# seobbro/TTA-depth-completion

Measured on AMD Instinct MI355X. Metric: TTA frames/sec (fwd+loss+bwd+Adam) at 352x1216, higher is better.
Workload: dtype mixed: real frames' forward (the scored depth) f32 storage + bf16x3 MFMA arithmetic; no_grad proxy pass and all data gradients bf16 storage + single bf16 MFMA; fp32 accumulate everywhere; loss / Adam / adapted parameters fp32 (include/ptta.h PTTA_DTYPE_MIXED)

## Files before the change

include/ptta.h:

```cpp
#ifndef PTTA_H
#define PTTA_H
#include <stdint.h>
#ifdef __cplusplus
extern "C" {
#endif

typedef struct ptta_ctx* ptta_handle;
typedef void* ptta_stream;

enum { PTTA_BACKBONE_MSG_CHN = 0, PTTA_BACKBONE_NLSPN = 1, PTTA_BACKBONE_COSTDCNET = 2 };
enum { PTTA_DTYPE_F32 = 0, PTTA_DTYPE_MIXED = 1,
       PTTA_MIXED_KEEP_PROXY = 0x100, PTTA_MIXED_KEEP_BACKWARD = 0x200, PTTA_MIXED_KEEP_HEADS = 0x400,
       PTTA_MIXED_BWD_ROUNDED_W = 0x800 };
enum { PTTA_META_1LAYER = 0, PTTA_META_2LAYERS = 1 };
enum { PTTA_NLSPN_LEGACY_OFFSET = 0x100,
       PTTA_NLSPN_SYNCBN_ADAPT = 0x200,
       PTTA_SYNCBN_ADAPT = 0x200 };

typedef struct {
    float lr, beta1, beta2, eps, weight_decay;
    float w_sparse_depth, w_smoothness, w_cos;
    float max_input_depth;
    float max_predict_depth;
} ptta_hparams;
// ... 76 lines not shown
int ptta_head_set_form(ptta_handle h, int form);

int ptta_crop_flip(const float* src, float* dst, int n, int channels, int height, int width, int crop_height, int crop_width,
                   const int32_t* start_y, const int32_t* start_x, const uint8_t* hflip, const uint8_t* vflip, ptta_stream s);

int ptta_rotate(const float* src, float* dst, int n, int channels, int height, int width, const uint8_t* do_rotate, const float* angle_deg,
                int bilinear, ptta_stream s);
int ptta_resize_crop(const float* src, float* dst, int n, int channels, int height, int width, const uint8_t* do_resize,
                     const int32_t* resize_height, const int32_t* resize_width, const int32_t* start_y, const int32_t* start_x,
                     int bilinear, int scale_depth, ptta_stream s);
int ptta_photometric(const float* src, float* dst, int n, int height, int width, const uint8_t* do_brightness, const float* f_brightness,
                     const uint8_t* do_contrast, const float* f_contrast, const uint8_t* do_saturation, const float* f_saturation,
                     double* scratch, ptta_stream s);

int ptta_photometric_full(const float* src, float* dst, int n, int height, int width, const uint8_t* do_brightness, const float* f_brightness,
                          const uint8_t* do_contrast, const float* f_contrast, const uint8_t* do_gamma, const float* f_gamma,
                          const uint8_t* do_hue, const float* f_hue, const uint8_t* do_saturation, const float* f_saturation,
                          double* scratch, ptta_stream s);
int ptta_add_noise(const float* src, const float* noise, float* dst, int n, int channels, int height, int width, const uint8_t* do_noise,
                   float spread, int uniform, ptta_stream s);
int ptta_remove_patches(const float* src, float* dst, int n, int channels, int height, int width, const uint8_t* do_remove,
                        const uint8_t* selected, const int32_t* patch_height, const int32_t* patch_width, ptta_stream s);
int ptta_crop_pad(const float* src, float* dst, int n, int channels, int height, int width, const uint8_t* do_crop_pad,
                  const int32_t* start_y, const int32_t* start_x, const int32_t* end_y, const int32_t* end_x,
                  const int32_t* pad_top, const int32_t* pad_left, int padding_mode, float fill, ptta_stream s);
int ptta_resize_pad(const float* src, float* dst, int n, int channels, int height, int width, const uint8_t* do_resize_pad,
                    const int32_t* resize_height, const int32_t* resize_width, const int32_t* pad_top, const int32_t* pad_left,
                    int bilinear, int padding_mode, float fill, ptta_stream s);

typedef int (*ptta_allreduce_fn)(void* user, double* exchange_buf, long long count, ptta_stream s);
int ptta_set_stat_sync(ptta_handle h, ptta_allreduce_fn fn, void* user, double* exchange_buf, int64_t capacity, int world_size);

int ptta_rccl_unique_id(void* id128_host);
int ptta_rccl_comm_create(const void* id128_host, int rank, int world_size, void** comm_out_host);
int ptta_rccl_comm_destroy(void* comm);
int ptta_rccl_allreduce_mean_f32(void* comm, float* buf, int64_t count, ptta_stream s);
const char* ptta_rccl_last_error(void);
int ptta_set_stat_sync_rccl(ptta_handle h, void* comm, double* exchange_buf, int64_t capacity, int world_size);
int ptta_set_grad_sync_rccl(ptta_handle h, void* comm);

int ptta_set_graph(ptta_handle h, int enable);

int ptta_set_option(ptta_handle h, const char* key, int value);
int ptta_get_option(ptta_handle h, const char* key, int* value_host);

int ptta_profile(ptta_handle h, int enable);
int ptta_profile_read(ptta_handle h, int klass, double* ms_total_host, double* alg_bytes_host, double* macs_host,
                      int64_t* launches_host, ptta_stream s);

int ptta_debug_tensor(ptta_handle h, const char* name, float* dst, int64_t capacity, int64_t* numel_host, ptta_stream s);
int ptta_op_conv32(const float* in_nhwc, const float* weight, const float* bias, float* out_nhwc,
                   int b, int hin, int win, int mode, int relu_in, int in_major, int flip, int dtype, int naive,
                   ptta_stream s);
int ptta_op_gwgrad(const float* x_nhwc, const float* gy_nhwc, float* gw, float* gb, int b, int h, int w, int ci, int co, int impl,
                   int reps, float* us_per_call_host, ptta_stream s);
#define PTTA_GCONV_S1 0
#define PTTA_GCONV_S2 1
#define PTTA_GCONV_T2 2
#define PTTA_GCONV_VERT 1
#define PTTA_GCONV_X1_W2 2
#define PTTA_GCONV_DGRAD 4
int ptta_op_gconv(const float* x0, int c0, int ld0, const float* x1, int c1, int ld1, const float* weight, const float* bias, float* y,
                  int co, int ldy, int b, int hin, int win, int hout, int wout, int k, int geom, int act, int accumulate, int impl,
                  int flags, int six_b, int x1_from_b, int stat_npass, double* stat_host, int* form_host, ptta_stream s);
#define PTTA_GBN_TRAIN 0
#define PTTA_GBN_EVAL 1
#define PTTA_GBN_BACKWARD 2
typedef struct ptta_gbn_view { float* p; int c; int ld; } ptta_gbn_view;
typedef struct ptta_gbn_args {
    int mode, b, h, w, npass, act, act_first, res_relu, acc_gx, acc_gres, world, nblocks_in, repeats;
    float eps, momentum;
    ptta_gbn_view x, res, y, g, gx, gres;
    const float* gamma; const float* beta; const float* part_in;
    float* st; float* rm; float* rv; long long* nbt; float* st_eval; float* dgamma; float* dbeta;
} ptta_gbn_args;
int ptta_op_gbn(const ptta_gbn_args* a, ptta_stream s);
int ptta_op_conv32_chain(const float* in_nhwc, const float* weight, const float* bias, float* buf_a, float* buf_b, const float* aux,
                         int b, int h, int w, int relu_in, int epi_flags, int reps, int replays, float* us_per_launch_host, ptta_stream s);
#define PTTA_ABI_VERSION 2
int ptta_version(void);

#ifdef __cplusplus
}
#endif
#endif
```

tta-depth-completion_amd/csrc/conv_small.hip:

```cpp
#include "ptta_common.h"
#include "ptta_kernels.h"

template <typename T>
struct ConvInP {
    Plane pl[3]; int zero_from_b;
    const float* w;
    Epi<T> epi;
    int B, H, W;
};

template <typename T, int CIN>
__global__ __launch_bounds__(256) void conv_in_mfma_kernel(ConvInP<T> p) {
    constexpr int K = 9 * CIN;
    constexpr int NS = (K + 1) / 2;
    const int lane = threadIdx.x & 63;
    const int i = lane & 31, h = lane >> 5;
    const int wave = __builtin_amdgcn_readfirstlane((int)(threadIdx.x >> 6));
    float w[NS];
#pragma unroll
    for (int s = 0; s < NS; ++s) w[s] = p.w[s * 64 + lane];

    const int nseg = (p.W + 31) >> 5;
    const long nitems = (long)p.B * nseg * p.H;
    const float sy = up_scale(p.H >> 1, p.H), sx = up_scale(p.W >> 1, p.W);
// ... 146 lines not shown
void ptta_pack_conv_in(const float* src, int cin_total, int cin_first, int cin, int transpose_flip,
                       float* wfrag, float* wcanon, hipStream_t s) {
    hipLaunchKernelGGL(pack_conv_in_kernel, dim3(4), dim3(256), 0, s, src, cin_total, cin_first, cin,
                       transpose_flip, wfrag, wcanon);
}

template <typename T>
static int launch_conv_in_t(const ConvInArgs& a, hipStream_t s) {
    ConvInP<T> p;
    for (int c = 0; c < 3; ++c) { p.pl[c] = a.pl[c]; if (p.pl[c].nb < 1) p.pl[c].nb = 1; }
    p.zero_from_b = a.zero_from_b;
    p.epi.bias = a.bias;
    p.epi.up = (const T*)a.up; p.epi.up_nb = a.up_nb > 0 ? a.up_nb : 1;
    p.epi.mask = (const T*)a.mask; p.epi.mask_nb = a.mask_nb > 0 ? a.mask_nb : 1;
    p.epi.add1 = (const T*)a.add1; p.epi.add1_nb = a.add1_nb > 0 ? a.add1_nb : 1;
    p.epi.add2 = nullptr; p.epi.add2_nb = 1;
    p.epi.out_raw = (T*)a.out_raw; p.epi.out_sum = (T*)a.out_sum;
    p.epi.mask_bits = a.mask_bits;
    if (sizeof(T) == 4 && a.a_bits && a.a_bits_nb > 0 && !a.naive) { p.epi.bits_out = a.a_bits; p.epi.bits_nb = a.a_bits_nb; p.epi.bits_sum = 0; }
    if (sizeof(T) == 2 && a.mask && !a.mask_bits) return -22;
    p.B = a.B; p.H = a.H; p.W = a.W;
    if (a.naive) {
        p.w = a.wcanon;
        const long total = (long)p.B * p.H * p.W * 32;
        int blocks = (int)((total + 255) / 256); if (blocks > 8192) blocks = 8192;
        hipLaunchKernelGGL((conv_in_naive_kernel<T>), dim3(blocks), dim3(256), 0, s, p, a.cin);
    } else {
        p.w = a.wfrag;
        if (!a.up && !a.add1) {
            const long tiles = (long)p.B * ((p.W + 31) / 32) * ((p.H + CI_TH - 1) / CI_TH);
            const int blocks = (int)(tiles > 2048 ? 2048 : tiles);
#define CL_(C) do { if (a.mask) hipLaunchKernelGGL((conv_in_lds_kernel<T, C, true>), dim3(blocks), dim3(256), 0, s, p); \
                    else hipLaunchKernelGGL((conv_in_lds_kernel<T, C, false>), dim3(blocks), dim3(256), 0, s, p); } while (0)
            if (a.cin == 1) CL_(1); else if (a.cin == 2) CL_(2); else CL_(3);
#undef CL_
            PTTA_CHECK_LAUNCH();
            return 0;
        }
        const long items = (long)p.B * ((p.W + 31) / 32) * p.H;
        long blocks = (items + 3) / 4; if (blocks > 2048) blocks = 2048;
        if (a.cin == 1) hipLaunchKernelGGL((conv_in_mfma_kernel<T, 1>), dim3((int)blocks), dim3(256), 0, s, p);
        else if (a.cin == 2) hipLaunchKernelGGL((conv_in_mfma_kernel<T, 2>), dim3((int)blocks), dim3(256), 0, s, p);
        else hipLaunchKernelGGL((conv_in_mfma_kernel<T, 3>), dim3((int)blocks), dim3(256), 0, s, p);
    }
    PTTA_CHECK_LAUNCH();
    return 0;
}

int ptta_launch_conv_in(const ConvInArgs& a, hipStream_t s) {
    if (a.cin < 1 || a.cin > 3) return -22;
    return a.bf16 ? launch_conv_in_t<bf16_t>(a, s) : launch_conv_in_t<float>(a, s);
}

template <typename T, bool RELU>
__global__ __launch_bounds__(256) void conv_out1_lds_kernel(const T* __restrict__ in, int in_nb, const float* __restrict__ w,
                                                            const float* __restrict__ bias, const float* __restrict__ add,
                                                            int add_nb, float* __restrict__ out, int B, int H, int W) {
    constexpr int TH = 8, PW = 34, PH = TH + 2, NV = PH * PW * 8, NIT = (NV + 255) / 256;
    __shared__ float4 tile[NV];
    const int tid = threadIdx.x, lane = tid & 63, pl = lane >> 3, cq = lane & 7;
    const int wave = __builtin_amdgcn_readfirstlane((int)(tid >> 6));
    float4 wt[9];
#pragma unroll
    for (int t = 0; t < 9; ++t) wt[t] = *(const float4*)(w + t * 32 + 4 * cq);
    const float b0 = bias ? bias[0] : 0.f;
    const int ntx = (W + 31) >> 5, nty = (H + TH - 1) / TH;
    const long ntiles = (long)B * ntx * nty;
    for (long t = blockIdx.x; t < ntiles; t += gridDim.x) {
        long t_ = t;
        const int ty = (int)(t_ % nty); t_ /= nty;
        const int tx = (int)(t_ % ntx);
        const int b = (int)(t_ / ntx);
        const int y0 = ty * TH, x0 = tx << 5;
        const T* inb = in + (size_t)(b % in_nb) * H * W * 32;
        float4 v[NIT];
        unsigned okm = 0;
#pragma unroll
        for (int it = 0; it < NIT; ++it) {
            const int idx = min(tid + 256 * it, NV - 1);
            const int q = idx & 7, pix = idx >> 3;
            const int py = pix / PW, px = pix - py * PW;
            const int gy = y0 - 1 + py, gx = x0 - 1 + px;
            okm |= (gy >= 0 && gy < H && gx >= 0 && gx < W) ? (1u << it) : 0u;
            const T* src = inb + ((size_t)min(max(gy, 0), H - 1) * W + min(max(gx, 0), W - 1)) * 32 + 4 * q;
            if constexpr (sizeof(T) == 4) v[it] = *(const float4*)src; else v[it] = bf4_to_f4(*(const uint2*)src);
        }
#pragma unroll
        for (int it = 0; it < NIT; ++it) {
            const int idx = tid + 256 * it;
            float4 a = v[it];
            if (!((okm >> it) & 1u)) a = make_float4(0.f, 0.f, 0.f, 0.f);
            if (RELU) { a.x = fmaxf(a.x, 0.f); a.y = fmaxf(a.y, 0.f); a.z = fmaxf(a.z, 0.f); a.w = fmaxf(a.w, 0.f); }
            if (idx < NV) tile[idx] = a;
        }
        lds_barrier();
#pragma unroll
        for (int rr = 0; rr < 2; ++rr) {
            const int row = 2 * wave + rr, y = y0 + row;
            const int xs = x0 + cq * 8 + pl;
            const bool sok = cq < 4 && y < H && xs < W;
            const size_t o = (size_t)min(y, H - 1) * W + min(xs, W - 1);
            float addv = 0.f;
            if (add) addv = add[(size_t)(b % add_nb) * H * W + o];
            float res = 0.f;
#pragma unroll
            for (int pass = 0; pass < 4; ++pass) {
                const float4* base = tile + (row * PW + pass * 8 + pl) * 8 + cq;
                float acc = 0.f;
#pragma unroll
                for (int tap = 0; tap < 9; ++tap) {
                    const float4 a = base[((tap / 3) * PW + tap % 3) * 8];
                    acc = fmaf(a.x, wt[tap].x, acc); acc = fmaf(a.y, wt[tap].y, acc);
                    acc = fmaf(a.z, wt[tap].z, acc); acc = fmaf(a.w, wt[tap].w, acc);
                }
                acc += __shfl_xor(acc, 1); acc += __shfl_xor(acc, 2); acc += __shfl_xor(acc, 4);
                res = cq == pass ? acc : res;
            }
            if (sok) {
                float r = res + b0;
                if (add) r += addv;
                out[(size_t)b * H * W + o] = r;
            }
        }
        lds_barrier();
    }
}

__global__ void pack_conv_out1_kernel(const float* __restrict__ src, int cin_total, int cin_index, int from_conv_in, float* w) {
    const int idx = blockIdx.x * blockDim.x + threadIdx.x;
    if (idx >= 288) return;
    const int c = idx & 31, tap = idx >> 5;
    w[idx] = from_conv_in ? src[((size_t)c * cin_total + cin_index) * 9 + (8 - tap)] : src[(size_t)c * 9 + tap];
}

void ptta_pack_conv_out1(const float* src, int src_cin_total, int src_cin_index, int from_conv_in, float* w, hipStream_t s) {
    hipLaunchKernelGGL(pack_conv_out1_kernel, dim3(2), dim3(256), 0, s, src, src_cin_total, src_cin_index, from_conv_in, w);
}

int ptta_launch_conv_out1(const ConvOut1Args& a, hipStream_t s) {
    const int add_nb = a.add_nb > 0 ? a.add_nb : 1;
    const long tiles = (long)a.B * ((a.W + 31) / 32) * ((a.H + 7) / 8);
    const int tb = (int)(tiles < 768 ? tiles : 768);
#define LDS_(T, R) hipLaunchKernelGGL((conv_out1_lds_kernel<T, R>), dim3(tb), dim3(256), 0, s, (const T*)a.in, a.in_nb, a.w, a.bias, a.add, add_nb, a.out, a.B, a.H, a.W)
    if (a.bf16) { if (a.relu_in) LDS_(bf16_t, true); else LDS_(bf16_t, false); }
    else { if (a.relu_in) LDS_(float, true); else LDS_(float, false); }
#undef LDS_
    PTTA_CHECK_LAUNCH();
    return 0;
}
```

tta-depth-completion_amd/csrc/ptta_kernels.h:

```cpp
#pragma once
#include <hip/hip_runtime.h>
#include <cstdlib>
#include <cstring>
#include "ptta_common.h"

struct PttaCreateEnv { int naive = 0, exact = 0, graph = -1; };
inline PttaCreateEnv ptta_create_env() {
    PttaCreateEnv e;
    const char* v = getenv("PTTA_CONV_IMPL"); e.naive = (v && strcmp(v, "naive") == 0) ? 1 : 0;
    v = getenv("PTTA_ARITH"); e.exact = (v && strcmp(v, "exact") == 0) ? 1 : 0;
    v = getenv("PTTA_GRAPH"); e.graph = (v && (strcmp(v, "0") == 0 || strcmp(v, "1") == 0)) ? (v[0] - '0') : -1;
    return e;
}

struct ConvW {
    float* mf32;
    bf16_t* mbf16;
    bf16_t* mlo;
    float* canon;
};
struct Conv32Args {
    const void* in = nullptr; int in_nb = 1;
    const ConvW* w = nullptr;
    const float* bias = nullptr;
    const void* up = nullptr; int up_nb = 1;
    const void* mask = nullptr; int mask_nb = 1;
    const void* add1 = nullptr; int add1_nb = 1;
    const void* add2 = nullptr; int add2_nb = 1;
    void* out_raw = nullptr; void* out_sum = nullptr;
    int B = 1, Hin = 0, Win = 0;
    int mode = CONV_S1; int relu_in = 0; int bf16 = 0; int naive = 0;
    int x3 = 0;
    int w2 = 0;
    const uint32_t* mask_bits = nullptr;
    uint32_t* bits_out = nullptr; int bits_nb = 0; int bits_sum = 0;
};
void ptta_pack_conv32(const float* src, const ConvW& w, int in_major, int flip, hipStream_t s, int row_stride = 32, int col_off = 0);
int ptta_launch_conv32(const Conv32Args& a, hipStream_t s);
int ptta_launch_conv32_loop(const Conv32Args& a, void* buf_a, void* buf_b, int reps, unsigned* ctr, unsigned* base_io, int* err, int variant, hipStream_t s);

struct Plane { const float* p = nullptr; int nb = 1; long bstride = 0;
               int norm = 0; float div = 1.f, mean = 0.f, stdv = 1.f; };
struct ConvInArgs {
    Plane pl[3]; int cin = 1; int zero_from_b = 1 << 30;
    const float* wfrag = nullptr;
    const float* wcanon = nullptr;
    const float* bias = nullptr;
    const void* up = nullptr; int up_nb = 1;
    const void* mask = nullptr; int mask_nb = 1;
    const void* add1 = nullptr; int add1_nb = 1;
    void* out_raw = nullptr; void* out_sum = nullptr;
    int B = 1, H = 0, W = 0; int bf16 = 0; int naive = 0;
    const uint32_t* mask_bits = nullptr; uint32_t* a_bits = nullptr;
    int a_bits_nb = 0;
};
void ptta_pack_conv_in(const float* src, int cin_total, int cin_first, int cin, int transpose_flip,
                       float* wfrag, float* wcanon, hipStream_t s);
int ptta_launch_conv_in(const ConvInArgs& a, hipStream_t s);
int ptta_launch_conv32_first(const Conv32Args& a, const ConvInArgs& f, void* a_out, int a_nb, hipStream_t s);

struct ConvOut1Args {
    const void* in = nullptr; int in_nb = 1;
    const float* w = nullptr;
    const float* bias = nullptr;
    const float* add = nullptr; int add_nb = 1;
    float* out = nullptr;
    int B = 1, H = 0, W = 0; int relu_in = 0; int bf16 = 0;
};
void ptta_pack_conv_out1(const float* src, int src_cin_total, int src_cin_index, int from_conv_in, float* w, hipStream_t s);
int ptta_launch_conv_out1(const ConvOut1Args& a, hipStream_t s);

int ptta_launch_prep(const float* sparse, float max_input_depth, float* dclamp, float* d12, float* d14,
                     int N, int H, int W, hipStream_t s);
int ptta_launch_up2_1ch(const float* in, float* out, int B, int Hin, int Win, hipStream_t s);
int ptta_launch_up2T_1ch(const float* gout, float* gin, int B, int Hin, int Win, hipStream_t s);
int ptta_launch_up2T_32(const void* gout, const void* add, void* gin, int B, int Hin, int Win, int bf16, hipStream_t s);

int ptta_launch_outlier_removal(const float* sparse, const float* validity, float* sparse_out, float* validity_out,
                                int N, int H, int W, int ksize, float threshold, float* scratch, hipStream_t s);

typedef int (*ptta_allreduce_cb)(void* user, double* dev_buf, long long count, void* stream);
int ptta_rccl_sum_f64(void* comm, double* buf, long long count, hipStream_t s);
struct PttaStatSync {
    ptta_allreduce_cb fn = nullptr; void* user = nullptr;
    void* comm = nullptr;
    double* buf = nullptr; long cap = 0; int world = 1;
    bool on() const { return (fn || comm) && (world > 1 || comm); }
    int exchange(long long count, hipStream_t s) const {
        if (comm) return ptta_rccl_sum_f64(comm, buf, count, s);
        const int rc = fn(user, buf, count, (void*)s);
        return rc ? (rc < 0 ? rc : -rc) : 0;
    }
};
int ptta_stat_sync(const PttaStatSync* sy, float* part, int nblocks, int C, int npass, hipStream_t s);
int ptta_grad_mean_sync(const PttaStatSync* sy, float* g, long n, hipStream_t s);

struct GemmArgs {
    const void* A = nullptr; int a_bf16 = 0;
    const float* A2 = nullptr;
    const float* W = nullptr;
    const float* bias = nullptr;
    float* C = nullptr;
    int R = 0, K = 0, N = 0;
    int pro = 0;
    const float* pscale = nullptr; const float* pshift = nullptr;
    const float* pmean = nullptr; const float* pinv = nullptr;
    const float* pc1 = nullptr; const float* pc2 = nullptr;
    int epi = 0;
    const float* eH = nullptr;
    const float* escale = nullptr; const float* eshift = nullptr; const float* emean = nullptr; const float* einv = nullptr;
    float* part = nullptr;
    int x3 = 0; const bf16_t* Whi = nullptr; const bf16_t* Wlo = nullptr;
    const bf16_t* Wil = nullptr;
    const float* X = nullptr;
    const void* W0frag = nullptr;
    const float* b0 = nullptr;
    const bf16_t* W0hi = nullptr; const bf16_t* W0lo = nullptr;
    const bf16_t* W0thi = nullptr; const bf16_t* W0tlo = nullptr;
    float* P = nullptr;
    const float* Bref = nullptr; const float* rowstats = nullptr; const float* coef = nullptr;
// ... 196 lines not shown
```

tta-depth-completion_amd/csrc/ptta_ops.hip:

```cpp
#include "msgchn_ctx.h"
#include "gnet.h"

using namespace msgchn;

namespace {
struct ScratchConvW {
    ConvW w{};
    bool ok;
    ScratchConvW() {
        ok = hipMalloc((void**)&w.mf32, 9 * 4 * 64 * 4 * 4) == hipSuccess && hipMalloc((void**)&w.mbf16, 9 * 2 * 64 * 8 * 2) == hipSuccess &&
             hipMalloc((void**)&w.canon, 9216 * 4) == hipSuccess && hipMalloc((void**)&w.mlo, 9 * 2 * 64 * 8 * 2) == hipSuccess;
    }
    ~ScratchConvW() { (void)hipFree(w.mf32); (void)hipFree(w.mbf16); (void)hipFree(w.mlo); (void)hipFree(w.canon); }
    ScratchConvW(const ScratchConvW&) = delete;
    ScratchConvW& operator=(const ScratchConvW&) = delete;
};

__global__ void op_scale_f64_kernel(double* buf, long long n, double f) {
    for (long long i = (long long)blockIdx.x * blockDim.x + threadIdx.x; i < n; i += (long long)gridDim.x * blockDim.x) buf[i] *= f;
}
int op_gbn_exchange(void* user, double* buf, long long count, void* stream) {
    long long blocks = (count + 255) / 256; if (blocks > 1024) blocks = 1024; if (blocks < 1) blocks = 1;
    hipLaunchKernelGGL(op_scale_f64_kernel, dim3((int)blocks), dim3(256), 0, (hipStream_t)stream, buf, count, (double)*(const int*)user);
    return hipGetLastError() == hipSuccess ? 0 : -5;
// ... 17 lines not shown
                                    (hipStream_t)s);
}

static void dcn_args(DcnArgs& a, const float* input, const float* weight, const float* bias, const float* offset, const float* mask,
                     int b, int c, int h, int w, int c_out, int kh, int kw, int sh, int sw, int ph, int pw, int dh, int dw, int group, int dg) {
    a.in = input; a.weight = weight; a.bias = bias; a.offset = offset; a.mask = mask;
    a.B = b; a.C = c; a.H = h; a.W = w; a.Co = c_out; a.kh = kh; a.kw = kw; a.sh = sh; a.sw = sw; a.ph = ph; a.pw = pw;
    a.dh = dh; a.dw = dw; a.group = group; a.dg = dg;
}

int ptta_mdconv_forward(const float* input, const float* weight, const float* bias, const float* offset, const float* mask, float* output,
                        int b, int c, int h, int w, int c_out, int kh, int kw, int sh, int sw, int ph, int pw, int dh, int dw,
                        int group, int deformable_group, ptta_stream s) {
    if (!input || !weight || !offset || !mask || !output) return -22;
    DcnArgs a; dcn_args(a, input, weight, bias, offset, mask, b, c, h, w, c_out, kh, kw, sh, sw, ph, pw, dh, dw, group, deformable_group);
    a.out = output;
    return ptta_launch_dcn_forward(a, (hipStream_t)s);
}

int ptta_mdconv_backward(const float* input, const float* weight, const float* bias, const float* offset, const float* mask,
                         const float* grad_output, float* grad_input, float* grad_offset, float* grad_mask, float* grad_weight,
                         float* grad_bias, int b, int c, int h, int w, int c_out, int kh, int kw, int sh, int sw, int ph, int pw,
                         int dh, int dw, int group, int deformable_group, ptta_stream s) {
    if (!input || !weight || !offset || !mask || !grad_output) return -22;
    DcnArgs a; dcn_args(a, input, weight, bias, offset, mask, b, c, h, w, c_out, kh, kw, sh, sw, ph, pw, dh, dw, group, deformable_group);
    a.gout = grad_output; a.gin = grad_input; a.goff = grad_offset; a.gmask = grad_mask; a.gweight = grad_weight; a.gbias = grad_bias;
    return ptta_launch_dcn_backward(a, (hipStream_t)s);
}

int ptta_op_conv32(const float* in, const float* weight, const float* bias, float* out, int b, int hin, int win, int mode,
                   int relu_in, int in_major, int flip, int dtype, int naive, ptta_stream s_) {
    hipStream_t s = (hipStream_t)s_;
    ScratchConvW sw; ConvW& w = sw.w;
    void *tin = nullptr, *tout = nullptr;
    const int ho = mode == CONV_S1 ? hin : (mode == CONV_S2 ? hin / 2 : hin * 2), wo = mode == CONV_S1 ? win : (mode == CONV_S2 ? win / 2 : win * 2);
    const long nin = (long)b * hin * win * 32, nout = (long)b * ho * wo * 32;
    int rc = 0;
    if (!sw.ok || hipMalloc(&tin, nin * 2) != hipSuccess || hipMalloc(&tout, nout * 2) != hipSuccess) rc = -12;
    if (rc == 0) {
        ptta_pack_conv32(weight, w, in_major, flip, s);
        Conv32Args a; a.w = &w; a.bias = bias; a.B = b; a.Hin = hin; a.Win = win; a.mode = mode; a.relu_in = relu_in; a.naive = naive & 1; a.x3 = (naive >> 1) & 1;
        if (dtype != PTTA_DTYPE_F32) {
            from_f32_launch(in, (bf16_t*)tin, nin, s);
            a.in = tin; a.in_nb = b; a.out_raw = tout; a.bf16 = 1;
            rc = ptta_launch_conv32(a, s);
            to_f32_launch((const bf16_t*)tout, out, nout, s);
        } else {
            a.in = in; a.in_nb = b; a.out_raw = out; a.bf16 = 0;
            rc = ptta_launch_conv32(a, s);
        }
        (void)hipStreamSynchronize(s);
    }
    (void)hipFree(tin); (void)hipFree(tout);
    return rc;
}

int ptta_op_gwgrad(const float* x, const float* gy, float* gw, float* gb, int b, int h, int w, int ci, int co, int impl, int reps,
                   float* us_per_call_host, ptta_stream s_) {
    hipStream_t s = (hipStream_t)s_;
    if (!x || !gy || !gw || b < 1 || h < 1 || w < 1 || ci < 1 || co < 1 || ci > 256 || co > 256 || impl < 0 || impl > 2 || reps < 0 ||
        (reps > 0 && !us_per_call_host)) return -22;
    GView xv, gv;
    xv.p = (float*)x; xv.B = b; xv.H = h; xv.W = w; xv.C = ci; xv.ld = ci;
    gv.p = (float*)gy; gv.B = b; gv.H = h; gv.W = w; gv.C = co; gv.ld = co;
    const long P = (long)b * h * w;
    const size_t nm = (size_t)ptta_gwgrad_mfma_part_floats(P, ci, co), nn = (size_t)ptta_gwgrad_slabs(P) * (9 * ci * co + co);
    float* part = nullptr;
    if (hipMalloc((void**)&part, (impl == 2 ? nn : nm) * 4) != hipSuccess) return -12;
    auto run = [&]() {
        return impl == 0 ? ptta_launch_gwgrad_mfma(xv, gv, part, gw, gb, s)
                         : (impl == 1 ? ptta_launch_gwgrad_f32mfma(xv, gv, part, gw, gb, s) : ptta_launch_gwgrad(xv, gv, part, gw, gb, s));
    };
    int rc = run();
    if (!rc && reps > 0) {
        hipEvent_t e0 = nullptr, e1 = nullptr;
        if (hipEventCreate(&e0) != hipSuccess || hipEventCreate(&e1) != hipSuccess) rc = -5;
        if (!rc) {
            (void)hipEventRecord(e0, s);
            for (int r = 0; r < reps && !rc; ++r) rc = run();
            (void)hipEventRecord(e1, s);
            (void)hipEventSynchronize(e1);
            float ms = 0.f; (void)hipEventElapsedTime(&ms, e0, e1);
            *us_per_call_host = 1e3f * ms / (float)reps;
        }
        if (e0) (void)hipEventDestroy(e0);
        if (e1) (void)hipEventDestroy(e1);
    }
    if (hipStreamSynchronize(s) != hipSuccess && !rc) rc = -5;
    (void)hipFree(part);
    return rc;
}

int ptta_op_gconv(const float* x0, int c0, int ld0, const float* x1, int c1, int ld1, const float* weight, const float* bias, float* y, int co,
                  int ldy, int b, int hin, int win, int hout, int wout, int k, int geom, int act, int accumulate, int impl, int flags,
                  int six_b, int x1_from_b, int stat_npass, double* stat_host, int* form_host, ptta_stream s_) {
    hipStream_t s = (hipStream_t)s_;
    const bool vert = flags & PTTA_GCONV_VERT, dgrad = flags & PTTA_GCONV_DGRAD;
    if (!x0 || !weight || !y || b < 1 || hin < 1 || win < 1 || hout < 1 || wout < 1 || c0 < 1 || c1 < 0 || co < 1 || ld0 < c0 || ldy < co ||
        (c1 > 0) != (x1 != nullptr) || (c1 > 0 && ld1 < c1) || (k != 1 && k != 3) || geom < PTTA_GCONV_S1 || geom > PTTA_GCONV_T2 ||
        act < GACT_NONE || act > GACT_SIGMOID || impl < 0 || impl > 1 || (flags & ~7) || six_b < 0 || six_b > b || x1_from_b < 0 ||
        stat_npass < 0 || stat_npass > 2 || (accumulate & ~1)) return -22;
    if (vert && (k != 3 || geom != PTTA_GCONV_S1)) return -22;
    if (dgrad && (c1 > 0 || six_b > 0)) return -22;
    if (stat_npass > 0 && (!stat_host || geom != PTTA_GCONV_S1 || impl != 0 || dgrad || (b % stat_npass))) return -22;
    const int run = !dgrad ? geom : (geom == PTTA_GCONV_S2 ? PTTA_GCONV_T2 : (geom == PTTA_GCONV_T2 ? PTTA_GCONV_S2 : PTTA_GCONV_S1));
    const bool size_ok = run == PTTA_GCONV_S1 ? (hout == hin && wout == win)
// ... 225 lines not shown
```

tta-depth-completion_amd/proxytta/_lib.py:

```python
import ctypes
import os
from ctypes import POINTER, byref, c_char_p, c_float, c_int, c_int64, c_uint64, c_void_p


_HERE = os.path.dirname(os.path.abspath(__file__))
LIB_PATH = os.path.join(_HERE, 'libptta_hip.so')

PTTA_BACKBONE_MSG_CHN = 0
PTTA_BACKBONE_NLSPN = 1
PTTA_BACKBONE_COSTDCNET = 2
PTTA_NLSPN_LEGACY_OFFSET = 0x100
PTTA_NLSPN_SYNCBN_ADAPT = 0x200
PTTA_SYNCBN_ADAPT = 0x200
PTTA_META_1LAYER = 0
PTTA_META_2LAYERS = 1
PTTA_DTYPE_F32 = 0
PTTA_DTYPE_MIXED = 1
PTTA_HEAD_FORM_PLAIN = 0
PTTA_HEAD_FORM_SYNCBN = 1
PTTA_ABI_VERSION = 2
CONV_S1, CONV_S2, CONV_T2 = 0, 1, 2


class Hparams(ctypes.Structure):
# ... 28 lines not shown
    ('ptta_forward_eval', c_int, [_P, _P, _P, _P, _P]),
    ('ptta_loss_forward', c_int, [_P, _P, _P, _P, _P, _P, _P, c_int64, c_float, c_float, c_float, _P, _P]),
    ('ptta_loss_backward', c_int, [_P, _P, _P, _P, _P, _P, _P, c_int64, _P, _P, _P]),
    ('ptta_backward', c_int, [_P, _P, _P, _P, _P, _P]),
    ('ptta_set_grad', c_int, [_P, c_char_p, _P, c_int64, _P]),
    ('ptta_get_grad', c_int, [_P, c_char_p, _P, c_int64, _P]),
    ('ptta_adapted_count', c_int, [_P]),
    ('ptta_adapted_name', c_char_p, [_P, c_int, POINTER(c_int64)]),
    ('ptta_adapted_repeat', c_int, [_P, c_int]),
    ('ptta_adam_step', c_int, [_P, _P, _P, _P]),
    ('ptta_step', c_int, [_P, _P, _P, _P, _P, _P, _P, _P]),
    ('ptta_step_pipelined', c_int, [_P] * 5 + [c_uint64] + [_P] * 2 + [c_uint64] + [_P] * 3),
    ('ptta_pipeline_stream', c_int, [_P, POINTER(c_void_p)]),
    ('ptta_forward_eval_last', c_int, [_P, _P, _P]),
    ('ptta_outlier_removal', c_int, [_P, _P, _P, _P, c_int, c_int, c_int, c_int, c_float, _P, _P]),
    ('ptta_eval_metrics', c_int, [_P, _P, c_int64, c_float, c_float, _P, _P, _P]),
    ('ptta_mdconv_forward', c_int, [_P] * 6 + [c_int] * 15 + [_P]),
    ('ptta_mdconv_backward', c_int, [_P] * 11 + [c_int] * 15 + [_P]),
    ('ptta_set_image_norm', c_int, [_P, c_float, POINTER(c_float), POINTER(c_float)]),
    ('ptta_head_bind', c_int, [_P, c_char_p, _P, _P, _P]),
    ('ptta_head_set_hparams', c_int, [_P, c_float, c_float, c_float, c_float, c_float, c_float, c_int, _P]),
    ('ptta_head_reload', c_int, [_P, _P]),
    ('ptta_head_forward', c_int, [_P, _P, _P, c_int, _P, _P, _P]),
    ('ptta_head_backward', c_int, [_P, _P, _P]),
    ('ptta_head_adam_step', c_int, [_P, _P]),
    ('ptta_head_step', c_int, [_P, _P, _P, c_int, _P, _P]),
    ('ptta_head_get_grad', c_int, [_P, c_char_p, _P, c_int64, POINTER(c_int), _P]),
    ('ptta_head_set_form', c_int, [_P, c_int]),
    ('ptta_crop_flip', c_int, [_P, _P] + [c_int] * 6 + [_P] * 5),
    ('ptta_rotate', c_int, [_P, _P, c_int, c_int, c_int, c_int, _P, _P, c_int, _P]),
    ('ptta_resize_crop', c_int, [_P, _P, c_int, c_int, c_int, c_int, _P, _P, _P, _P, _P, c_int, c_int, _P]),
    ('ptta_photometric', c_int, [_P, _P, c_int, c_int, c_int, _P, _P, _P, _P, _P, _P, _P, _P]),
    ('ptta_photometric_full', c_int, [_P, _P, c_int, c_int, c_int] + [_P] * 12),
    ('ptta_add_noise', c_int, [_P, _P, _P, c_int, c_int, c_int, c_int, _P, c_float, c_int, _P]),
    ('ptta_remove_patches', c_int, [_P, _P, c_int, c_int, c_int, c_int, _P, _P, _P, _P, _P]),
    ('ptta_crop_pad', c_int, [_P, _P, c_int, c_int, c_int, c_int] + [_P] * 7 + [c_int, c_float, _P]),
    ('ptta_resize_pad', c_int, [_P, _P, c_int, c_int, c_int, c_int] + [_P] * 5 + [c_int, c_int, c_float, _P]),
    ('ptta_set_stat_sync', c_int, [_P, _P, _P, _P, c_int64, c_int]),
    ('ptta_rccl_unique_id', c_int, [_P]),
    ('ptta_rccl_comm_create', c_int, [_P, c_int, c_int, POINTER(c_void_p)]),
    ('ptta_rccl_comm_destroy', c_int, [_P]),
    ('ptta_rccl_allreduce_mean_f32', c_int, [_P, _P, c_int64, _P]),
    ('ptta_rccl_last_error', c_char_p, []),
    ('ptta_set_stat_sync_rccl', c_int, [_P, _P, _P, c_int64, c_int]),
    ('ptta_set_grad_sync_rccl', c_int, [_P, _P]),
    ('ptta_set_graph', c_int, [_P, c_int]),
    ('ptta_set_option', c_int, [_P, c_char_p, c_int]),
    ('ptta_get_option', c_int, [_P, c_char_p, POINTER(c_int)]),
    ('ptta_profile', c_int, [_P, c_int]),
    ('ptta_profile_read', c_int, [_P, c_int, POINTER(ctypes.c_double), POINTER(ctypes.c_double), POINTER(ctypes.c_double),
                                  POINTER(c_int64), _P]),
    ('ptta_debug_tensor', c_int, [_P, c_char_p, _P, c_int64, POINTER(c_int64), _P]),
    ('ptta_op_conv32', c_int, [_P, _P, _P, _P, c_int, c_int, c_int, c_int, c_int, c_int, c_int, c_int, c_int, _P]),
    ('ptta_op_conv32_chain', c_int, [_P] * 6 + [c_int] * 7 + [POINTER(c_float), _P]),
    ('ptta_op_gwgrad', c_int, [_P, _P, _P, _P] + [c_int] * 7 + [POINTER(c_float), _P]),
    ('ptta_op_gconv', c_int, [_P, c_int, c_int, _P, c_int, c_int, _P, _P, _P] + [c_int] * 16 + [POINTER(ctypes.c_double), POINTER(c_int), _P]),
    ('ptta_op_gbn', c_int, [POINTER(GbnArgs), _P]),
    ('ptta_version', c_int, []),
]

_lib = None


def load():
    global _lib
    if _lib is not None:
        return _lib
    import torch
    if not os.path.exists(LIB_PATH):
        raise RuntimeError('libptta_hip.so not found at %s: build it with `python -c "import '
                           '__graft_entry__ as g; g.build()"` — there is no CPU fallback' % LIB_PATH)
    lib = ctypes.CDLL(LIB_PATH)
    for name, res, args in SIGNATURES:
        fn = getattr(lib, name)
        fn.restype = res
        fn.argtypes = args
    have = lib.ptta_version()
    if have != PTTA_ABI_VERSION:
        raise RuntimeError('%s has ABI version %d, this binding is written against %d (include/ptta.h PTTA_ABI_VERSION): rebuild it with '
                           '`make -C tta-depth-completion_amd/csrc`' % (LIB_PATH, have, PTTA_ABI_VERSION))
    _lib = lib
    return lib


def check(lib, handle, rc, what):
    if rc != 0:
        msg = lib.ptta_last_error(handle).decode() if handle else ''
        raise RuntimeError('%s failed (%d): %s' % (what, rc, msg))


def ptr(t):
    if t is None:
        return None
    assert t.is_contiguous()
    return c_void_p(t.data_ptr())


__all__ = ['load', 'check', 'ptr', 'Hparams', 'GbnArgs', 'GbnView', 'SIGNATURES', 'LIB_PATH', 'byref']
```

tta-depth-completion_amd/proxytta/engine.py:

```python
import ctypes
from ctypes import byref, c_int, c_int64, c_void_p

import torch

from . import _lib
from ._lib import Hparams, check, ptr

ADAPTED = ('conv1_rgb_meta.weight', 'conv1_rgb_meta.bias')
_P2 = 'conv1_rgb_meta.conv1_meta.'
ADAPTED_2LAYERS = (_P2 + '0.0.weight', _P2 + '0.1.weight', _P2 + '0.1.bias', _P2 + '1.weight', _P2 + '1.bias',
                   _P2 + '2.weight', _P2 + '2.bias')


HEAD_PARAMS = tuple('%s.%s.%s' % (m, l, t) for m in ('proj', 'pred') for l in ('0', '1', '3') for t in ('weight', 'bias'))
HEAD_TARGETS = tuple('proj_t' + k[4:] for k in HEAD_PARAMS[:6])


def adapted_names(meta='1layer'):
    return ADAPTED_2LAYERS if meta == '2layers' else ADAPTED
_BOUND_SUFFIX = ('running_mean', 'running_var', 'num_batches_tracked')


def _stream():
    return c_void_p(torch.cuda.current_stream().cuda_stream)
# ... 355 lines not shown
        image = self._f32(image, (self.n, 3, self.h, self.w))
        sparse = self._f32(sparse, (self.n, 1, self.h, self.w))
        loss = torch.empty(1, device=image.device, dtype=torch.float32)
        self._chk(self.lib.ptta_head_step(self.handle, ptr(image), ptr(sparse), int(bool(reverse)), ptr(loss), _stream()), 'ptta_head_step')
        return loss

    def head_grad(self, name, like):
        has = c_int(0)
        out = torch.empty_like(like)
        self._chk(self.lib.ptta_head_get_grad(self.handle, name.encode(), ptr(out), out.numel(), byref(has), _stream()), 'ptta_head_get_grad')
        return out if has.value else None

    def set_graph(self, enable):
        self._chk(self.lib.ptta_set_graph(self.handle, int(bool(enable))), 'ptta_set_graph')

    def set_option(self, key, value):
        self._chk(self.lib.ptta_set_option(self.handle, key.encode(), int(value)), 'ptta_set_option(%s)' % key)

    def get_option(self, key):
        v = ctypes.c_int(0)
        self._chk(self.lib.ptta_get_option(self.handle, key.encode(), byref(v)), 'ptta_get_option(%s)' % key)
        return v.value

    def profile(self, enable):
        self._chk(self.lib.ptta_profile(self.handle, int(bool(enable))), 'ptta_profile')

    def profile_read(self, klass):
        ms, by, mc, n = ctypes.c_double(0), ctypes.c_double(0), ctypes.c_double(0), c_int64(0)
        self._chk(self.lib.ptta_profile_read(self.handle, int(klass), byref(ms), byref(by), byref(mc), byref(n), _stream()),
                  'ptta_profile_read')
        return ms.value, by.value, mc.value, n.value

    def debug_tensor(self, name):
        n = c_int64(0)
        self._chk(self.lib.ptta_debug_tensor(self.handle, name.encode(), None, 0, byref(n), _stream()), 'ptta_debug_tensor')
        out = torch.empty(n.value, device=self.device, dtype=torch.float32)
        self._chk(self.lib.ptta_debug_tensor(self.handle, name.encode(), ptr(out), n.value, byref(n), _stream()),
                  'ptta_debug_tensor')
        return out


def op_conv32(x_nhwc, weight, bias, mode, relu_in=False, in_major=False, flip=False, dtype='fp32', naive=False, x3=False):
    lib = _lib.load()
    b, h, w, _ = x_nhwc.shape
    ho, wo = {0: (h, w), 1: (h // 2, w // 2), 2: (2 * h, 2 * w)}[mode]
    out = torch.empty((b, ho, wo, 32), device=x_nhwc.device, dtype=torch.float32)
    rc = lib.ptta_op_conv32(ptr(x_nhwc.contiguous()), ptr(weight.contiguous()), ptr(bias), ptr(out), b, h, w, mode,
                            int(relu_in), int(in_major), int(flip), 0 if dtype == 'fp32' else 1, int(bool(naive)) | (2 if x3 else 0), _stream())
    if rc != 0:
        raise RuntimeError('ptta_op_conv32 failed (%d)' % rc)
    return out


GWGRAD_IMPLS = {'default': 0, 'fp32_mfma': 1, 'naive': 2}


def op_gwgrad(x_nhwc, gy_nhwc, impl='default', with_bias=True, reps=0):
    lib = _lib.load()
    b, h, w, ci = x_nhwc.shape
    co = gy_nhwc.shape[3]
    assert tuple(gy_nhwc.shape[:3]) == (b, h, w)
    x_nhwc, gy_nhwc = x_nhwc.float().contiguous(), gy_nhwc.float().contiguous()
    gw = torch.empty((co, ci, 3, 3), device=x_nhwc.device, dtype=torch.float32)
    gb = torch.empty((co,), device=x_nhwc.device, dtype=torch.float32) if with_bias else None
    us = ctypes.c_float(0.0)
    rc = lib.ptta_op_gwgrad(ptr(x_nhwc), ptr(gy_nhwc), ptr(gw), ptr(gb), b, h, w, ci, co,
                            GWGRAD_IMPLS[impl], int(reps), byref(us), _stream())
    if rc != 0:
        raise RuntimeError('ptta_op_gwgrad failed (%d)' % rc)
    return gw, gb, (us.value if reps > 0 else None)


GCONV_GEOMS = {'s1': 0, 's2': 1, 't2': 2}
GCONV_ACTS = {'none': 0, 'relu': 1, 'lrelu': 2, 'sigmoid': 3}
GCONV_IMPLS = {'mfma': 0, 'direct': 1}
GCONV_FORMS = {-1: None, 0: 'plain', 1: 'nco2', 2: 'ksplit'}


def op_gconv(x0, weight, y, x1=None, bias=None, k=3, geom='s1', act='none', accumulate=False, impl='mfma', vert=False, six_b=0,
             x1_from_b=None, x1_w2=False, dgrad=False, stat_npass=0):
    lib = _lib.load()

    def view(t):
        b, h, w, c = t.shape
        ld = t.stride(2)
        assert t.dtype == torch.float32 and t.stride(3) == 1 and t.stride(1) == w * ld and t.stride(0) == h * w * ld and ld >= c
        return c_void_p(t.data_ptr()), c, ld
    b, hin, win, _ = x0.shape
    hout, wout = y.shape[1], y.shape[2]
    assert y.shape[0] == b and (x1 is None or tuple(x1.shape[:3]) == (b, hin, win))
    p0, c0, ld0 = view(x0)
    p1, c1, ld1 = view(x1) if x1 is not None else (None, 0, 0)
    py, co, ldy = view(y)
    stats = (ctypes.c_double * (stat_npass * 2 * co))() if stat_npass else None
    form = c_int(-1)
    flags = (1 if vert else 0) | (2 if x1_w2 else 0) | (4 if dgrad else 0)
    rc = lib.ptta_op_gconv(p0, c0, ld0, p1, c1, ld1, ptr(weight.contiguous()), ptr(bias), py, co, ldy, b, hin, win, hout, wout, k,
                           GCONV_GEOMS[geom], GCONV_ACTS[act], int(bool(accumulate)), GCONV_IMPLS[impl], flags, int(six_b),
                           (1 << 30) if x1_from_b is None else int(x1_from_b), int(stat_npass), stats, byref(form), _stream())
    if rc != 0:
        raise RuntimeError('ptta_op_gconv failed (%d)' % rc)
    st = torch.tensor(list(stats), dtype=torch.float64).view(stat_npass, 2, co) if stat_npass else None
    return GCONV_FORMS[form.value], st


GBN_MODES = {'train': 0, 'eval': 1, 'backward': 2}
# ... 38 lines not shown
```

Baseline: 820.0.

## Restructure conv_out1 kernel with prefetch, bf16 LDS tile, row-pair reuse and contiguous tile chunks

The single-output 3x3 conv kernel now issues global loads for the next tile before computing the current one, so load latency overlaps with compute. For bf16 input the LDS tile is stored as bf16, halving shared-memory use. Each wave computes two output rows at once from four input rows, reusing loaded LDS values across rows. Tiles are split into contiguous chunks per block group, and the grid is sized by residency via launch_bounds occupancy hints. A standalone op entry point is added for testing. The risks are higher register pressure and an extra bf16 rounding of the fp32 path? No: only the narrow path is rounded, and it was already bf16.

```diff
diff --git a/include/ptta.h b/include/ptta.h
--- a/include/ptta.h
+++ b/include/ptta.h
@@ -152,6 +152,8 @@
 int ptta_op_conv32(const float* in_nhwc, const float* weight, const float* bias, float* out_nhwc,
                    int b, int hin, int win, int mode, int relu_in, int in_major, int flip, int dtype, int naive,
                    ptta_stream s);
+int ptta_op_conv_out1(const void* in_nhwc, int narrow, int in_nb, const float* w_packed, const float* bias, const float* add, int add_nb,
+                      float* out, int relu_in, int b, int h, int w, int max_blocks, ptta_stream s);
 int ptta_op_gwgrad(const float* x_nhwc, const float* gy_nhwc, float* gw, float* gb, int b, int h, int w, int ci, int co, int impl,
                    int reps, float* us_per_call_host, ptta_stream s);
 #define PTTA_GCONV_S1 0
diff --git a/tta-depth-completion_amd/csrc/conv_small.hip b/tta-depth-completion_amd/csrc/conv_small.hip
--- a/tta-depth-completion_amd/csrc/conv_small.hip
+++ b/tta-depth-completion_amd/csrc/conv_small.hip
@@ -222,12 +222,24 @@
     return a.bf16 ? launch_conv_in_t<bf16_t>(a, s) : launch_conv_in_t<float>(a, s);
 }
 
+#define CO1_BLOCKS_PER_CU_F32 3
+#define CO1_BLOCKS_PER_CU_NARROW 4
+template <typename T> struct Co1Piece { typedef float4 type; };
+template <> struct Co1Piece<bf16_t> { typedef uint2 type; };
+__device__ __forceinline__ float4 co1_widen(float4 v) { return v; }
+template <int M> __device__ __forceinline__ float co1_xor(float v) {
+    if constexpr (M == 4) return __int_as_float(__builtin_amdgcn_ds_swizzle(__float_as_int(v), 0x101F));
+    else return quad_xchg(v, M == 2);
+}
+__device__ __forceinline__ float4 co1_widen(uint2 v) { return bf4_to_f4(v); }
+
 template <typename T, bool RELU>
-__global__ __launch_bounds__(256) void conv_out1_lds_kernel(const T* __restrict__ in, int in_nb, const float* __restrict__ w,
+__global__ __launch_bounds__(256, sizeof(T) == 2 ? CO1_BLOCKS_PER_CU_NARROW : CO1_BLOCKS_PER_CU_F32) void conv_out1_lds_kernel(const T* __restrict__ in, int in_nb, const float* __restrict__ w,
                                                             const float* __restrict__ bias, const float* __restrict__ add,
                                                             int add_nb, float* __restrict__ out, int B, int H, int W) {
+    typedef typename Co1Piece<T>::type P;
     constexpr int TH = 8, PW = 34, PH = TH + 2, NV = PH * PW * 8, NIT = (NV + 255) / 256;
-    __shared__ float4 tile[NV];
+    __shared__ P tile[NV];
     const int tid = threadIdx.x, lane = tid & 63, pl = lane >> 3, cq = lane & 7;
     const int wave = __builtin_amdgcn_readfirstlane((int)(tid >> 6));
     float4 wt[9];
@@ -236,15 +248,29 @@
     const float b0 = bias ? bias[0] : 0.f;
     const int ntx = (W + 31) >> 5, nty = (H + TH - 1) / TH;
     const long ntiles = (long)B * ntx * nty;
-    for (long t = blockIdx.x; t < ntiles; t += gridDim.x) {
-        long t_ = t;
+    const int nch = min((int)gridDim.x, 8), chunk = blockIdx.x % nch;
+    const int step = ((int)gridDim.x - chunk + nch - 1) / nch;
+    const long t_end = ntiles * (chunk + 1) / nch;
+    long t = ntiles * chunk / nch + blockIdx.x / nch;
+    if (t >= t_end) return;
+
+    P v[NIT];
+    unsigned okm;
+    float addv[2];
+    int b, y0, x0;
+    auto issue = [&](long t_) {
         const int ty = (int)(t_ % nty); t_ /= nty;
         const int tx = (int)(t_ % ntx);
-        const int b = (int)(t_ / ntx);
-        const int y0 = ty * TH, x0 = tx << 5;
+        b = (int)(t_ / ntx);
+        y0 = ty * TH; x0 = tx << 5;
+        {
+            const float* ab = add ? add + (size_t)(b % add_nb) * H * W : w;
+#pragma unroll
+            for (int rr = 0; rr < 2; ++rr)
+                addv[rr] = ab[add ? (size_t)min(y0 + 2 * wave + rr, H - 1) * W + min(x0 + cq * 8 + pl, W - 1) : (size_t)0];
+        }
         const T* inb = in + (size_t)(b % in_nb) * H * W * 32;
-        float4 v[NIT];
-        unsigned okm = 0;
+        okm = 0;
 #pragma unroll
         for (int it = 0; it < NIT; ++it) {
             const int idx = min(tid + 256 * it, NV - 1);
@@ -252,46 +278,63 @@
             const int py = pix / PW, px = pix - py * PW;
             const int gy = y0 - 1 + py, gx = x0 - 1 + px;
             okm |= (gy >= 0 && gy < H && gx >= 0 && gx < W) ? (1u << it) : 0u;
-            const T* src = inb + ((size_t)min(max(gy, 0), H - 1) * W + min(max(gx, 0), W - 1)) * 32 + 4 * q;
-            if constexpr (sizeof(T) == 4) v[it] = *(const float4*)src; else v[it] = bf4_to_f4(*(const uint2*)src);
-        }
+            v[it] = *(const P*)(inb + ((size_t)min(max(gy, 0), H - 1) * W + min(max(gx, 0), W - 1)) * 32 + 4 * q);
+        }
+    };
+    issue(t);
+    for (;;) {
+        const int cb = b, cy0 = y0, cx0 = x0;
+        const float cadd[2] = {addv[0], addv[1]};
 #pragma unroll
         for (int it = 0; it < NIT; ++it) {
             const int idx = tid + 256 * it;
-            float4 a = v[it];
+            float4 a = co1_widen(v[it]);
             if (!((okm >> it) & 1u)) a = make_float4(0.f, 0.f, 0.f, 0.f);
             if (RELU) { a.x = fmaxf(a.x, 0.f); a.y = fmaxf(a.y, 0.f); a.z = fmaxf(a.z, 0.f); a.w = fmaxf(a.w, 0.f); }
-            if (idx < NV) tile[idx] = a;
+            if (idx < NV) {
+                if constexpr (sizeof(T) == 4) tile[idx] = a;
+                else tile[idx] = make_uint2((__float_as_uint(a.x) >> 16) | (__float_as_uint(a.y) & 0xffff0000u),
+                                            (__float_as_uint(a.z) >> 16) | (__float_as_uint(a.w) & 0xffff0000u));
+            }
         }
         lds_barrier();
+        const bool more = t + step < t_end;
+        if (more) { t += step; issue(t); }
+        float res[2] = {0.f, 0.f};
+#pragma unroll
+        for (int pass = 0; pass < 4; ++pass) {
+            const P* base = tile + ((2 * wave) * PW + pass * 8 + pl) * 8 + cq;
+            float acc0 = 0.f, acc1 = 0.f;
+#pragma unroll
+            for (int r = 0; r < 4; ++r)
+#pragma unroll
+                for (int dx = 0; dx < 3; ++dx) {
+                    const float4 a = co1_widen(base[(r * PW + dx) * 8]);
+                    if (r < 3) {
+                        const float4 k = wt[r * 3 + dx];
+                        acc0 = fmaf(a.x, k.x, acc0); acc0 = fmaf(a.y, k.y, acc0); acc0 = fmaf(a.z, k.z, acc0); acc0 = fmaf(a.w, k.w, acc0);
+                    }
+                    if (r > 0) {
+                        const float4 k = wt[(r - 1) * 3 + dx];
+                        acc1 = fmaf(a.x, k.x, acc1); acc1 = fmaf(a.y, k.y, acc1); acc1 = fmaf(a.z, k.z, acc1); acc1 = fmaf(a.w, k.w, acc1);
+                    }
+                }
+            acc0 += co1_xor<1>(acc0); acc0 += co1_xor<2>(acc0); acc0 += co1_xor<4>(acc0);
+            acc1 += co1_xor<1>(acc1); acc1 += co1_xor<2>(acc1); acc1 += co1_xor<4>(acc1);
+            res[0] = cq == pass ? acc0 : res[0];
+            res[1] = cq == pass ? acc1 : res[1];
+        }
 #pragma unroll
         for (int rr = 0; rr < 2; ++rr) {
-            const int row = 2 * wave + rr, y = y0 + row;
-            const int xs = x0 + cq * 8 + pl;
-            const bool sok = cq < 4 && y < H && xs < W;
-            const size_t o = (size_t)min(y, H - 1) * W + min(xs, W - 1);
-            float addv = 0.f;
-            if (add) addv = add[(size_t)(b % add_nb) * H * W + o];
-            float res = 0.f;
-#pragma unroll
-            for (int pass = 0; pass < 4; ++pass) {
-                const float4* base = tile + (row * PW + pass * 8 + pl) * 8 + cq;
-                float acc = 0.f;
-#pragma unroll
-                for (int tap = 0; tap < 9; ++tap) {
-                    const float4 a = base[((tap / 3) * PW + tap % 3) * 8];
-                    acc = fmaf(a.x, wt[tap].x, acc); acc = fmaf(a.y, wt[tap].y, acc);
-                    acc = fmaf(a.z, wt[tap].z, acc); acc = fmaf(a.w, wt[tap].w, acc);
-                }
-                acc += __shfl_xor(acc, 1); acc += __shfl_xor(acc, 2); acc += __shfl_xor(acc, 4);
-                res = cq == pass ? acc : res;
-            }
-            if (sok) {
-                float r = res + b0;
-                if (add) r += addv;
-                out[(size_t)b * H * W + o] = r;
-            }
-        }
+            const int y = cy0 + 2 * wave + rr;
+            const int xs = cx0 + cq * 8 + pl;
+            if (cq < 4 && y < H && xs < W) {
+                float r = res[rr] + b0;
+                if (add) r += cadd[rr];
+                out[((size_t)cb * H + y) * W + xs] = r;
+            }
+        }
+        if (!more) break;
         lds_barrier();
     }
 }
@@ -310,8 +353,12 @@
 int ptta_launch_conv_out1(const ConvOut1Args& a, hipStream_t s) {
     const int add_nb = a.add_nb > 0 ? a.add_nb : 1;
     const long tiles = (long)a.B * ((a.W + 31) / 32) * ((a.H + 7) / 8);
-    const int tb = (int)(tiles < 768 ? tiles : 768);
-#define LDS_(T, R) hipLaunchKernelGGL((conv_out1_lds_kernel<T, R>), dim3(tb), dim3(256), 0, s, (const T*)a.in, a.in_nb, a.w, a.bias, a.add, add_nb, a.out, a.B, a.H, a.W)
+    if (tiles < 1) return -22;
+    const long resident = 256 * (a.bf16 ? CO1_BLOCKS_PER_CU_NARROW : CO1_BLOCKS_PER_CU_F32);
+    long tb = tiles < 8 ? tiles : 8 * ((tiles + 7) / 8);
+    if (tb > resident) tb = resident;
+    if (a.max_blocks > 0) tb = a.max_blocks;
+#define LDS_(T, R) hipLaunchKernelGGL((conv_out1_lds_kernel<T, R>), dim3((unsigned)tb), dim3(256), 0, s, (const T*)a.in, a.in_nb, a.w, a.bias, a.add, add_nb, a.out, a.B, a.H, a.W)
     if (a.bf16) { if (a.relu_in) LDS_(bf16_t, true); else LDS_(bf16_t, false); }
     else { if (a.relu_in) LDS_(float, true); else LDS_(float, false); }
 #undef LDS_
diff --git a/tta-depth-completion_amd/csrc/ptta_kernels.h b/tta-depth-completion_amd/csrc/ptta_kernels.h
--- a/tta-depth-completion_amd/csrc/ptta_kernels.h
+++ b/tta-depth-completion_amd/csrc/ptta_kernels.h
@@ -66,6 +66,7 @@
     const float* add = nullptr; int add_nb = 1;
     float* out = nullptr;
     int B = 1, H = 0, W = 0; int relu_in = 0; int bf16 = 0;
+    int max_blocks = 0;
 };
 void ptta_pack_conv_out1(const float* src, int src_cin_total, int src_cin_index, int from_conv_in, float* w, hipStream_t s);
 int ptta_launch_conv_out1(const ConvOut1Args& a, hipStream_t s);
diff --git a/tta-depth-completion_amd/csrc/ptta_ops.hip b/tta-depth-completion_amd/csrc/ptta_ops.hip
--- a/tta-depth-completion_amd/csrc/ptta_ops.hip
+++ b/tta-depth-completion_amd/csrc/ptta_ops.hip
@@ -93,6 +93,17 @@
         (void)hipStreamSynchronize(s);
     }
     (void)hipFree(tin); (void)hipFree(tout);
+    return rc;
+}
+
+int ptta_op_conv_out1(const void* in, int narrow, int in_nb, const float* w, const float* bias, const float* add, int add_nb, float* out,
+                      int relu_in, int b, int h, int wd, int max_blocks, ptta_stream s_) {
+    hipStream_t s = (hipStream_t)s_;
+    if (!in || !w || !out || b < 1 || h < 1 || wd < 1 || in_nb < 1 || in_nb > b || (add && (add_nb < 1 || add_nb > b)) || max_blocks < 0) return -22;
+    ConvOut1Args a; a.in = in; a.in_nb = in_nb; a.w = w; a.bias = bias; a.add = add; a.add_nb = add ? add_nb : 1; a.out = out;
+    a.B = b; a.H = h; a.W = wd; a.relu_in = relu_in != 0; a.bf16 = narrow != 0; a.max_blocks = max_blocks;
+    int rc = ptta_launch_conv_out1(a, s);
+    if (hipStreamSynchronize(s) != hipSuccess && !rc) rc = -5;
     return rc;
 }
 
diff --git a/tta-depth-completion_amd/proxytta/_lib.py b/tta-depth-completion_amd/proxytta/_lib.py
--- a/tta-depth-completion_amd/proxytta/_lib.py
+++ b/tta-depth-completion_amd/proxytta/_lib.py
@@ -104,6 +104,7 @@
                                   POINTER(c_int64), _P]),
     ('ptta_debug_tensor', c_int, [_P, c_char_p, _P, c_int64, POINTER(c_int64), _P]),
     ('ptta_op_conv32', c_int, [_P, _P, _P, _P, c_int, c_int, c_int, c_int, c_int, c_int, c_int, c_int, c_int, _P]),
+    ('ptta_op_conv_out1', c_int, [_P, c_int, c_int, _P, _P, _P, c_int, _P] + [c_int] * 5 + [_P]),
     ('ptta_op_conv32_chain', c_int, [_P] * 6 + [c_int] * 7 + [POINTER(c_float), _P]),
     ('ptta_op_gwgrad', c_int, [_P, _P, _P, _P] + [c_int] * 7 + [POINTER(c_float), _P]),
     ('ptta_op_gconv', c_int, [_P, c_int, c_int, _P, c_int, c_int, _P, _P, _P] + [c_int] * 16 + [POINTER(ctypes.c_double), POINTER(c_int), _P]),
diff --git a/tta-depth-completion_amd/proxytta/engine.py b/tta-depth-completion_amd/proxytta/engine.py
--- a/tta-depth-completion_amd/proxytta/engine.py
+++ b/tta-depth-completion_amd/proxytta/engine.py
@@ -431,6 +431,19 @@
     return out
 
 
+def op_conv_out1(x_nhwc, w_packed, bias=None, add=None, relu_in=False, batch=None, max_blocks=0):
+    lib = _lib.load()
+    in_nb, h, w, c = x_nhwc.shape
+    assert c == 32 and x_nhwc.dtype in (torch.float32, torch.bfloat16) and tuple(w_packed.shape) == (9, 32)
+    b = in_nb if batch is None else int(batch)
+    out = torch.empty((b, h, w), device=x_nhwc.device, dtype=torch.float32)
+    rc = lib.ptta_op_conv_out1(ptr(x_nhwc.contiguous()), int(x_nhwc.dtype == torch.bfloat16), in_nb, ptr(w_packed.contiguous()), ptr(bias),
+                               ptr(add), add.shape[0] if add is not None else 1, ptr(out), int(relu_in), b, h, w, int(max_blocks), _stream())
+    if rc != 0:
+        raise RuntimeError('ptta_op_conv_out1 failed (%d)' % rc)
+    return out
+
+
 GWGRAD_IMPLS = {'default': 0, 'fp32_mfma': 1, 'naive': 2}
 
 
```

Result: no change. 817.9 (-0.2%).
